# ViV99/slam-experiments

Hardware: NVIDIA B200
Metric: hamming_pairs_per_sec (higher is better)
Workload: dtype u8

## Files before the change

### slam_experiments_b200/csrc/hm_tc.cu

```cuda
#include <math.h>
#include <stdlib.h>

#include <mutex>
#include <type_traits>

#include <cuda_fp16.h>

#include "hm_common.cuh"
#include "hm_tcgen05.cuh"

#ifndef HM_F4_TILE_N
#define HM_F4_TILE_N 128
#endif

namespace hm {

namespace {

constexpr int kRowBlock = 128;
constexpr int kMBlocks = 2;
constexpr int kBlockM = kRowBlock * kMBlocks;
constexpr int kSlabBytes = kRowBlock * 128;
constexpr int kPadRows = HM_PREPARED_TILE_ROWS;
constexpr int kTmemCols = 512;
constexpr uint32_t kSpinLimit = 1u << 26;

static_assert(kPadRows % kBlockM == 0, "prepared padding must cover whole query blocks");

struct CoreI8 {
    using Acc = int;
    static constexpr int kSlabs = 2;
    static constexpr int kRowBytes = HM_PREPARED_ROW_BYTES;
    static constexpr int kTileN = 128;
    static constexpr int kStages = 4;
    static constexpr int kUnits = 4;
    static constexpr int kColSplit = 1;
    static constexpr bool kRegisterHandover = false;
    static constexpr bool kScales = false;
    static constexpr int kPrologueTiles = 45;
    static __device__ __forceinline__ Acc lowest() { return INT_MIN; }
    static __device__ __forceinline__ Acc from_bits(uint32_t x) { return (int)x; }
    static __device__ __forceinline__ Acc max3(Acc a, Acc b, Acc c) { return __vimax3_s32(a, b, c); }
    static __device__ __forceinline__ Acc max2(Acc a, Acc b) { return max(a, b); }
    static __device__ __forceinline__ bool valid(Acc v) { return v >= -256; }
    static __device__ __forceinline__ unsigned distance(Acc v) { return (unsigned)((256 - v) >> 1); }
    static __device__ __forceinline__ unsigned encode(Acc v) { return (unsigned)(v + 257); }
    static __device__ __forceinline__ Acc floor_from(unsigned e) { return (int)e - 259; }
    static __device__ __forceinline__ uint32_t pack2(uint32_t lo, uint32_t hi) { return ((uint32_t)max((int)lo, -32768) & 0xFFFFu) | ((uint32_t)max((int)hi, -32768) << 16); }
    static __device__ __forceinline__ Acc unpack(uint32_t p, int hi) { return hi ? (int)p >> 16 : (int)(short)(p & 0xFFFFu); }
    static constexpr uint32_t kLowestBits = 0x80000000u;
};

struct CoreF4 {
    using Acc = float;
    static constexpr int kSlabs = 1;
    static constexpr int kRowBytes = HM_PREPARED_F4_ROW_BYTES;
    static constexpr int kTileN = HM_F4_TILE_N;
#ifndef HM_F4_STAGES
#define HM_F4_STAGES 6
#endif
    static constexpr int kStages = HM_F4_TILE_N == 96 ? 10 : HM_F4_TILE_N == 64 ? 14 : HM_F4_STAGES;
#ifndef HM_F4_UNITS
#define HM_F4_UNITS (HM_F4_TILE_N == 96 ? 5 : HM_F4_TILE_N == 64 ? 7 : 3)
#endif
    static constexpr int kUnits = HM_F4_UNITS;
    static constexpr int kColSplit = 2;
    static constexpr bool kRegisterHandover = true;
    static constexpr bool kScales = true;
    static constexpr int kPrologueTiles = 90;
    static __device__ __forceinline__ Acc lowest() { return -INFINITY; }
    static __device__ __forceinline__ Acc from_bits(uint32_t x) { return __uint_as_float(x); }
    static __device__ __forceinline__ Acc max3(Acc a, Acc b, Acc c) { return fmaxf(fmaxf(a, b), c); }
    static __device__ __forceinline__ Acc max2(Acc a, Acc b) { return fmaxf(a, b); }
    static __device__ __forceinline__ bool valid(Acc v) { return v >= -256.0f; }
    static __device__ __forceinline__ unsigned distance(Acc v) { return (unsigned)((256 - (int)v) >> 1); }
    static __device__ __forceinline__ unsigned encode(Acc v) { return (unsigned)((int)v + 257); }
    static __device__ __forceinline__ Acc floor_from(unsigned e) { return (float)((int)e - 259); }
    static __device__ __forceinline__ uint32_t pack2(uint32_t lo, uint32_t hi)
    {
        const __half2 h = __floats2half2_rn(__uint_as_float(lo), __uint_as_float(hi));
        return *reinterpret_cast<const uint32_t*>(&h);
    }
    static __device__ __forceinline__ Acc unpack(uint32_t p, int hi)
    {
        const __half2 h = *reinterpret_cast<const __half2*>(&p);
        return hi ? __high2float(h) : __low2float(h);
    }
    static constexpr uint32_t kLowestBits = 0xFF800000u;
};

template <class C> __host__ __device__ constexpr int row_block_bytes() { return kRowBlock * C::kRowBytes; }
template <class C> __host__ __device__ constexpr int a_bytes() { return kMBlocks * row_block_bytes<C>(); }
template <class C> __host__ __device__ constexpr int b_stage_bytes() { return C::kTileN * C::kRowBytes; }
template <class C> __host__ __device__ constexpr int epilogue_warps() { return 4 * kMBlocks * C::kColSplit; }
template <class C> __host__ __device__ constexpr int control_warps() { return C::kRegisterHandover ? 4 : 2; }
template <class C> __host__ __device__ constexpr int threads() { return 32 * (control_warps<C>() + epilogue_warps<C>()); }
constexpr int kHandoverBytes = kBlockM * 16;
constexpr int kBarrierBytes = 512;
template <class C> __host__ __device__ constexpr int smem_bytes() { return 1024 + a_bytes<C>() + C::kStages * b_stage_bytes<C>() + kBarrierBytes + kHandoverBytes; }
static_assert((2 * CoreF4::kStages + 1 + 2 * CoreF4::kUnits) * 8 + 16 <= kBarrierBytes, "barrier block");
static_assert((2 * CoreI8::kStages + 1 + 2 * CoreI8::kUnits) * 8 + 16 <= kBarrierBytes, "barrier block");
__host__ __device__ constexpr int ct_gcd(int a, int b) { return b == 0 ? a : ct_gcd(b, a % b); }
template <class C> __host__ __device__ constexpr int issuer_period() { return C::kStages / ct_gcd(C::kStages, C::kUnits) * C::kUnits; }
constexpr int kScaleCols = 32;
constexpr int kScaleCol = kTmemCols - kScaleCols;
static_assert(CoreF4::kUnits * CoreF4::kTileN <= kScaleCol, "accumulator units must end before the scale factors");

struct PrepareParams {
    const uint8_t* bits;
    long long n, stride, batch_stride;
    long long padded_rows;
    uint8_t* out;
};

__global__ void __launch_bounds__(256) hm_prepare_kernel(const PrepareParams P)
{
    const long long chunks_per_problem = P.padded_rows * 16;
    const long long o = (long long)blockIdx.x * blockDim.x + threadIdx.x;
    if (o >= chunks_per_problem) return;
    const int b = blockIdx.y;
    const long long rb = o >> 11;
    const int rem = (int)(o & 2047);
    const int slab = rem >> 10;
    const int rem2 = rem & 1023;
    const int rr = (rem2 >> 3) & 7;
    const int r = ((rem2 >> 6) << 3) | rr;
    const int c = (rem2 & 7) ^ rr;
// ... 130 lines not shown
#if HM_TC_TRACE
    unsigned slow;
#endif
};

__device__ __forceinline__ void bounded_wait(uint64_t* bar, uint32_t parity, int* error_flag)
{
    uint32_t spins = 0;
    while (!ptx::mbar_try_wait(bar, parity)) {
        if (++spins > kSpinLimit) {
            if (error_flag) atomicExch(error_flag, 1);
            __trap();
        }
    }
}

__device__ __forceinline__ void bounded_wait_addr(uint32_t bar_addr, uint32_t parity, int* error_flag)
{
    uint32_t spins = 0;
    while (!ptx::mbar_try_wait_addr(bar_addr, parity)) {
        if (++spins > kSpinLimit) {
            if (error_flag) atomicExch(error_flag, 1);
            __trap();
        }
    }
}

#define HM_R8(a, o) "+r"(a[o]), "+r"(a[o + 1]), "+r"(a[o + 2]), "+r"(a[o + 3]), "+r"(a[o + 4]), "+r"(a[o + 5]), "+r"(a[o + 6]), "+r"(a[o + 7])
#define HM_R32(a) HM_R8(a, 0), HM_R8(a, 8), HM_R8(a, 16), HM_R8(a, 24)
__device__ __forceinline__ void tmem_ld_fence4(uint32_t (&a)[32], uint32_t (&b)[32], uint32_t (&c)[32], uint32_t (&d)[32])
{
    asm volatile("tcgen05.wait::ld.sync.aligned;\n" : HM_R32(a), HM_R32(b), HM_R32(c), HM_R32(d) : : "memory");
}
__device__ __forceinline__ void tmem_ld_fence48(uint32_t (&a)[32], uint32_t (&b)[16])
{
    asm volatile("tcgen05.wait::ld.sync.aligned;\n" : HM_R32(a), HM_R8(b, 0), HM_R8(b, 8) : : "memory");
}
__device__ __forceinline__ void tmem_ld_fence64(uint32_t (&a)[64])
{
    asm volatile("tcgen05.wait::ld.sync.aligned;\n" : HM_R8(a, 0), HM_R8(a, 8), HM_R8(a, 16), HM_R8(a, 24), HM_R8(a, 32), HM_R8(a, 40), HM_R8(a, 48), HM_R8(a, 56) : : "memory");
}

template <class C, int kMode, int kGroups = 4>
__device__ __forceinline__ void scan_chunk(const uint32_t* r, unsigned colbase, Top2<typename C::Acc>& s)
{
    using Acc = typename C::Acc;
    static_assert(kGroups == 2 || kGroups == 4 || kGroups == 8, "8-column groups per compare");
    Acc gm[kGroups];
#pragma unroll
    for (int g = 0; g < kGroups; ++g) {
        const int o = g * 8;
        gm[g] = C::max3(C::max3(C::from_bits(r[o]), C::from_bits(r[o + 1]), C::from_bits(r[o + 2])),
                        C::max3(C::from_bits(r[o + 3]), C::from_bits(r[o + 4]), C::from_bits(r[o + 5])),
                        C::max2(C::from_bits(r[o + 6]), C::from_bits(r[o + 7])));
    }
    Acc m;
    if constexpr (kGroups == 8) m = C::max3(C::max3(gm[0], gm[1], gm[2]), C::max3(gm[3], gm[4], gm[5]), C::max2(gm[6], gm[7]));
    else if constexpr (kGroups == 4) m = C::max3(gm[0], gm[1], C::max2(gm[2], gm[3]));
    else m = C::max2(gm[0], gm[1]);
    constexpr bool kFloor = kMode == 1, kTop1 = kMode == 2;
    if (m > (kFloor ? s.f : kTop1 ? s.v1 : s.v2)) {
#if HM_TC_TRACE
        s.slow += 1;
#endif
#pragma unroll
        for (int g = 0; g < kGroups; ++g) {
            const Acc x = gm[g];
            if (x > (kFloor ? s.f : kTop1 ? s.v1 : s.v2)) {
                const int o = g * 8;
                const uint32_t p0 = C::pack2(r[o], r[o + 1]), p1 = C::pack2(r[o + 2], r[o + 3]);
                const uint32_t p2 = C::pack2(r[o + 4], r[o + 5]), p3 = C::pack2(r[o + 6], r[o + 7]);
                const unsigned idx = colbase + o;
                if (kTop1 || x > s.v1) {
                    if (!kTop1) {
                        s.v2 = s.v1; s.i2 = s.i1;
                        s.sb[0] = s.sa[0]; s.sb[1] = s.sa[1]; s.sb[2] = s.sa[2]; s.sb[3] = s.sa[3];
                    }
                    s.v1 = x; s.i1 = idx;
                    s.sa[0] = p0; s.sa[1] = p1; s.sa[2] = p2; s.sa[3] = p3;
                } else {
                    s.v2 = x; s.i2 = idx;
                    s.sb[0] = p0; s.sb[1] = p1; s.sb[2] = p2; s.sb[3] = p3;
                }
                if (kFloor) s.f = C::max2(s.v2, s.f);
            }
        }
    }
}

template <class C, int kN>
__device__ __forceinline__ void mask_tail(uint32_t* r, unsigned colbase, unsigned limit)
{
    if (colbase + kN > limit) {
#pragma unroll
        for (int j = 0; j < kN; ++j)
            if (colbase + j >= limit) r[j] = C::kLowestBits;
    }
}

#ifndef HM_ARRIVE_ELECT
#define HM_ARRIVE_ELECT 1
#endif
#ifndef HM_SCAN_FLAT64
#define HM_SCAN_FLAT64 1
#endif
#ifndef HM_FLOOR_DENSE_TILES
#define HM_FLOOR_DENSE_TILES 32
#endif
#ifndef HM_FLOOR_LATE_MASK
#define HM_FLOOR_LATE_MASK 15
#endif

#ifndef HM_F4_A_TMEM
#define HM_F4_A_TMEM 0
#endif
constexpr int kATmemCol = 384;
constexpr int kATmemColsPerBlock = 32;

template <class C>
__device__ __forceinline__ void issue_half(int h, uint32_t a_block, uint32_t b_stage, uint32_t tmem_d, uint32_t idesc,
                                           uint32_t tmem_sf)
{
    constexpr int kHalf = C::kSlabs * 2;
#pragma unroll
    for (int jj = 0; jj < kHalf; ++jj) {
        const int j = h * kHalf + jj;
        const int slab = j >> 2, k = j & 3;
        const uint64_t db = ptx::kmajor_sw128_desc_from_lo(b_stage + ((slab * kSlabBytes + k * 32) >> 4));
        if constexpr (C::kScales && HM_F4_A_TMEM) {
            ptx::mma_mxf4_ts(tmem_d, a_block + 8 * j, db, idesc, tmem_sf, tmem_sf + kScaleCols / 2, j != 0);
        } else {
            const uint64_t da = ptx::kmajor_sw128_desc_from_lo(a_block + ((slab * kSlabBytes + k * 32) >> 4));
            if constexpr (C::kScales) ptx::mma_mxf4_ss(tmem_d, da, db, idesc, tmem_sf, tmem_sf + kScaleCols / 2, j != 0);
            else                      ptx::mma_i8_ss(tmem_d, da, db, idesc, j != 0);
        }
    }
}

// ... 21 lines not shown
    uint64_t* tmem_empty_bar = tmem_full_bar + kUnits;
    uint32_t* tmem_base_slot = reinterpret_cast<uint32_t*>(tmem_empty_bar + kUnits);
    uint32_t* smem_base_slot = tmem_base_slot + 2;
    ulonglong2* handover = reinterpret_cast<ulonglong2*>(smem + kABytes + kStages * kBStageBytes + kBarrierBytes);

    const int warp = __shfl_sync(0xffffffffu, threadIdx.x >> 5, 0);
    const int lane = threadIdx.x & 31;
    if (threadIdx.x == 0) cta_mark(P, 0);
    if (threadIdx.x == 0 && (blockIdx.x | blockIdx.y | blockIdx.z) == 0 && P.clock_probe) {
        unsigned long long t;
        asm volatile("mov.u64 %0, %%globaltimer;" : "=l"(t));
        P.clock_probe[0] = (long long)t;
        P.clock_probe[1] = clock64();
    }
    const int qb = blockIdx.x;
    const int split = blockIdx.y;
    const int b = blockIdx.z;

    const uint32_t cs = ptx::cluster_nctarank();
    const uint32_t crank = ptx::cluster_ctarank();
    const uint16_t cmask = (uint16_t)((1u << cs) - 1);
    const bool has_a = qb < P.q_blocks_valid;
    auto rows_present = [&]() -> long long { return P.nq_dyn ? min((long long)__ldg(P.nq_dyn + b), P.nq) : P.nq; };
    if (P.nq_dyn && (long long)(qb - (int)crank) * kBlockM >= rows_present()) return;

    const int tile_begin = split * P.tiles_per_split;
    const int tile_end = min(tile_begin + P.tiles_per_split, P.ntiles);
    const int my_tiles = tile_end - tile_begin;

    constexpr int kProducerWarp = kIssuerLast ? epilogue_warps<C>() : 0;
    constexpr int kIssuerWarp = kIssuerLast ? epilogue_warps<C>() + 1 : 1;
    constexpr int kFirstEpiWarp = kIssuerLast ? 0 : 2;
    static_assert(kIssuerLast || !C::kRegisterHandover, "the control warps must form the last warpgroup");
    static_assert(!C::kRegisterHandover || (epilogue_warps<C>() == 16 && threads<C>() == 640),
                  "the register budget (4 x 32 + 16 x 112 = 20 x 96) assumes 20 warps launched at 96 registers");
    if (warp == kProducerWarp && lane == 0) {
        *smem_base_slot = ptx::smem_u32(smem);
        for (int i = 0; i < kStages; ++i) {
            ptx::mbar_init(&full_bar[i], 1);
            ptx::mbar_init(&empty_bar[i], cs);
        }
        ptx::mbar_init(a_full_bar, 1);
        for (int i = 0; i < kUnits; ++i) {
            ptx::mbar_init(&tmem_full_bar[i], 1);
            ptx::mbar_init(&tmem_empty_bar[i], 4 * C::kColSplit);
        }
        ptx::fence_barrier_init();
        ptx::fence_proxy_async();
    } else if (warp == kIssuerWarp) {
        ptx::tmem_alloc(tmem_base_slot, kTmemCols);
        ptx::tmem_relinquish();
    }
    ptx::tc_fence_before();
    if (cs > 1) ptx::cluster_sync();
    else __syncthreads();
    ptx::tc_fence_after();
    const uint32_t tmem_base = *tmem_base_slot;

    if constexpr (C::kScales) {
        if (warp >= kFirstEpiWarp && warp < kFirstEpiWarp + 4) {
            uint32_t ones[32];
#pragma unroll
            for (int i = 0; i < 32; ++i) ones[i] = 0x7F7F7F7Fu;
            const uint32_t taddr = tmem_base + ((uint32_t)((warp & 3) * 32) << 16) + kScaleCol;
            static_assert(kScaleCols == 32, "one x32 store per lane quarter");
            ptx::tmem_st_32x32(taddr, ones);
            ptx::tmem_st_wait();
        }
// ... 27 lines not shown
                            const uint4 v = row[c ^ (r & 7)];
                            words[4 * c] = v.x; words[4 * c + 1] = v.y; words[4 * c + 2] = v.z; words[4 * c + 3] = v.w;
                        }
                    }
                }
                ptx::tmem_st_32x32(tmem_base + ((uint32_t)(wq * 32) << 16) + kATmemCol + wblk * kATmemColsPerBlock, words);
                ptx::tmem_st_wait();
            }
        } else if (P.qbits) {
            const uint8_t* qsrc = P.qbits + (long long)b * P.q_bits_batch_stride;
            const int* qidx = P.q_index ? P.q_index + (long long)b * P.q_index_batch_stride : nullptr;
            const long long nq_eff = rows_present();
            for (int o = threadIdx.x; o < kBlockM * 8; o += blockDim.x) {
                const int blk = o >> 10, rem = o & 1023;
                const int rr = (rem >> 3) & 7;
                const int r = ((rem >> 6) << 3) | rr;
                const int c = (rem & 7) ^ rr;
                const long long qrow = (long long)qb * kBlockM + blk * kRowBlock + r;
                uint4 v = make_uint4(0, 0, 0, 0);
                if (qrow < nq_eff) {
                    const long long srow = qidx ? (long long)__ldg(qidx + qrow) : qrow;
                    v = expand_bits_e2m1(*reinterpret_cast<const unsigned*>(qsrc + srow * P.q_bits_stride + c * 4));
                }
                reinterpret_cast<uint4*>(smem_a)[o] = v;
            }
            ptx::fence_proxy_async();
        }
        ptx::tc_fence_before();
        __syncthreads();
        ptx::tc_fence_after();
    }

    if (threadIdx.x == 0) cta_mark(P, 1);
    ulonglong2 my_keys = make_ulonglong2(kNoMatch, kNoMatch);
    long long my_row = -1;
    int my_row_in_cta = 0;

    auto run_producer = [&]() {
        if (lane == 0) {
            if (has_a && !P.qbits && !(C::kScales && HM_F4_A_TMEM)) {
                const uint8_t* qsrc = P.qprep + ((long long)b * P.q_padded + (long long)qb * kBlockM) * C::kRowBytes;
                ptx::mbar_arrive_expect_tx(a_full_bar, kABytes);
                ptx::bulk_g2s(smem_a, qsrc, kABytes, a_full_bar);
            }
            const uint8_t* tsrc = P.tprep + (long long)b * P.t_padded * C::kRowBytes;
            const uint32_t piece = kBStageBytes / cs;
            for (int i = 0; i < (HM_TC_EXPERIMENT >= 5 ? 0 : my_tiles); ++i) {
                const int stage = i % kStages;
                const uint32_t use = i / kStages;
#if HM_TC_EXPERIMENT < 4
                bounded_wait(&empty_bar[stage], (use & 1) ^ 1, P.error_flag);
#endif
                trace_mark(P, i, 0);
                ptx::mbar_arrive_expect_tx(&full_bar[stage], kBStageBytes);
                uint8_t* dst = smem_b + stage * kBStageBytes + crank * piece;
                const uint8_t* src = tsrc + (long long)(tile_begin + i) * kBStageBytes + crank * piece;
                if (cs > 1) ptx::bulk_g2s_multicast(dst, src, piece, &full_bar[stage], cmask);
                else        ptx::bulk_g2s(dst, src, piece, &full_bar[stage]);
            }
        }
    };
    auto run_issuer = [&]() {
        const bool leader = ptx::elect_one();
        const uint32_t idesc = C::kScales ? ptx::make_mxf4_idesc(kRowBlock, kTileN) : ptx::make_i8_idesc(kRowBlock, kTileN);
        constexpr bool kATmem = C::kScales && HM_F4_A_TMEM;
        const uint32_t a_addr = kATmem ? tmem_base + kATmemCol : ptx::smem_u32(smem_a) >> 4;
        constexpr uint32_t kABlockStep = kATmem ? (uint32_t)kATmemColsPerBlock : (uint32_t)(kRowBlockBytes >> 4);
        const uint32_t b_addr = ptx::smem_u32(smem_b) >> 4;
        const uint32_t tmem_sf = tmem_base + kScaleCol;
// ... 41 lines not shown
                    if (leader) issue_half<C>(0, a_addr + kABlockStep, b_stage, tmem_base + unit_b * kTileN, idesc, tmem_sf);
                    ready0 = false;
                    if (base + j + 1 < my_tiles) {
                        const int n = j + 1;
#if HM_TC_EXPERIMENT >= 4
                        ready0 = true;
#else
                        ready0 = __all_sync(0xffffffffu,
                                            ptx::mbar_test_wait(&full_bar[n % kStages], sphase ^ ((n / kStages) & 1))
#if HM_TC_EXPERIMENT < 3
                                            && ptx::mbar_test_wait(&tmem_empty_bar[(2 * n) % kUnits], (((2 * n) / kUnits) & 1) ^ 1)
#endif
                                            );
#endif
                    }
                    if (leader) {
                        issue_half<C>(1, a_addr + kABlockStep, b_stage, tmem_base + unit_b * kTileN, idesc, tmem_sf);
#if HM_TC_EXPERIMENT == 6 || HM_COMMIT_MODE == 1
                        ptx::tc_commit(&tmem_full_bar[unit_a]);
#endif
                        ptx::tc_commit(&tmem_full_bar[unit_b]);
                        if (cs > 1) ptx::tc_commit_multicast(&empty_bar[stage], cmask);
                        else        ptx::tc_commit(&empty_bar[stage]);
                    }
                }
            }
            sphase ^= (kPeriod / kStages) & 1;
        }
        __syncwarp();
    };
    auto run_epilogue = [&]() {
        constexpr int kCols = kTileN / C::kColSplit;
        const int quarter = warp & 3;
        const int mblk = ((warp - kFirstEpiWarp) >> 2) & 1;
        const int half = (warp - kFirstEpiWarp) >> 3;
        const int row_in_cta = mblk * kRowBlock + quarter * 32 + lane;
        const long long row = (long long)qb * kBlockM + row_in_cta;
        Top2<Acc> s;
        s.v1 = s.v2 = C::lowest();
        s.i1 = s.i2 = 0;
#pragma unroll
        for (int e = 0; e < 4; ++e) s.sa[e] = s.sb[e] = 0;
        s.f = C::floor_from(0);
#if HM_TC_TRACE
        s.slow = 0;
#endif
        unsigned floor_code = 0;
        const long long first_row = (long long)tile_begin * kTileN;
        const unsigned limit = (unsigned)min((long long)my_tiles * kTileN, P.nt - first_row);
        const uint32_t bars_addr = ptx::lds_volatile_u32(ptx::smem_u32(smem_base_slot)) + kABytes + kStages * kBStageBytes;
        const uint32_t unit_full_addr = bars_addr + (2 * kStages + 1) * 8;
        const uint32_t unit_empty_addr = unit_full_addr + kUnits * 8;
        int unit = mblk;
        uint32_t unit_use = 0;
        unsigned floor_pending = 0;
        auto refresh_floor = [&](int i) {
            if constexpr (kFloor) {
                if (i < HM_FLOOR_DENSE_TILES || (i & HM_FLOOR_LATE_MASK) == 0) {
                    floor_code = max(floor_code, floor_pending);
                    s.f = C::max2(s.f, C::floor_from(floor_code));
                    if (row < P.nq) {
                        unsigned* floor_ptr = P.row_floor + ((long long)b * P.nq + row);
                        const unsigned e = C::valid(s.v2) ? C::encode(s.v2) : 0u;
                        if (e > floor_code) { atomicMax(floor_ptr, e); floor_code = e; }
                        floor_pending = __ldcg(floor_ptr);
                    }
                }
            }
        };
        auto process_tile = [&](int i) {
            bounded_wait_addr(unit_full_addr + unit * 8, unit_use & 1, P.error_flag);
#if HM_TC_TRACE == 2
            if (warp == kFirstEpiWarp && lane == 0 && (i == 8 || i == 32 || i == 64 || i == 192)) cta_mark(P, i == 8 ? 5 : i == 32 ? 6 : i == 64 ? 7 : 8);
#endif
            if (warp == kFirstEpiWarp && lane == 0) trace_mark(P, i, 3);
            if (warp == kFirstEpiWarp + 7 && lane == 0) trace_mark(P, i, 5);
            ptx::tc_fence_after();
            const uint32_t taddr = tmem_base + ((uint32_t)(quarter * 32) << 16) + unit * kTileN + half * kCols;
            const unsigned colbase = (unsigned)i * kTileN + half * kCols;
            if constexpr (C::kColSplit == 1) {
                uint32_t r0[32], r1[32], r2[32], r3[32];
                ptx::tmem_ld_32x32(taddr, r0);
                ptx::tmem_ld_32x32(taddr + 32, r1);
                ptx::tmem_ld_32x32(taddr + 64, r2);
                ptx::tmem_ld_32x32(taddr + 96, r3);
                refresh_floor(i);
                tmem_ld_fence4(r0, r1, r2, r3);
                ptx::tc_fence_before();
                __syncwarp();
                if (HM_ARRIVE_ELECT ? ptx::elect_one() : lane == 0) ptx::mbar_arrive_addr(unit_empty_addr + unit * 8);
                if (colbase + kCols > limit) {
                    mask_tail<C, 32>(r0, colbase, limit);
                    mask_tail<C, 32>(r1, colbase + 32, limit);
                    mask_tail<C, 32>(r2, colbase + 64, limit);
                    mask_tail<C, 32>(r3, colbase + 96, limit);
                }
                scan_chunk<C, kMode>(r0, colbase, s);
                scan_chunk<C, kMode>(r1, colbase + 32, s);
                scan_chunk<C, kMode>(r2, colbase + 64, s);
                scan_chunk<C, kMode>(r3, colbase + 96, s);
            } else {
                if constexpr (kCols == 64) {
                    uint32_t r[64];
#if HM_TC_EXPERIMENT < 2
                    ptx::tmem_ld_32x64(taddr, r);
                    refresh_floor(i);
                    tmem_ld_fence64(r);
#endif
                    ptx::tc_fence_before();
                    __syncwarp();
                    if (HM_ARRIVE_ELECT ? ptx::elect_one() : lane == 0) ptx::mbar_arrive_addr(unit_empty_addr + unit * 8);
#if HM_TC_EXPERIMENT != 0
                    unit += 2;
                    if (unit >= kUnits) { unit -= kUnits; ++unit_use; }
                    return;
#endif
                    mask_tail<C, 64>(r, colbase, limit);
#if HM_SCAN_FLAT64
                    scan_chunk<C, kMode, 8>(r, colbase, s);
#else
                    scan_chunk<C, kMode>(r, colbase, s);
                    scan_chunk<C, kMode>(r + 32, colbase + 32, s);
#endif
                } else if constexpr (kCols == 32) {
                    uint32_t r[32];
                    ptx::tmem_ld_32x32(taddr, r);
                    refresh_floor(i);
                    asm volatile("tcgen05.wait::ld.sync.aligned;\n" : HM_R32(r) : : "memory");
                    ptx::tc_fence_before();
                    __syncwarp();
                    if (HM_ARRIVE_ELECT ? ptx::elect_one() : lane == 0) ptx::mbar_arrive_addr(unit_empty_addr + unit * 8);
                    mask_tail<C, 32>(r, colbase, limit);
                    scan_chunk<C, kMode>(r, colbase, s);
                } else {
                    static_assert(kCols == 64 || kCols == 48, "column split");
                    uint32_t r0[32], r1[16];
                    ptx::tmem_ld_32x32(taddr, r0);
                    ptx::tmem_ld_32x16(taddr + 32, r1);
                    refresh_floor(i);
                    tmem_ld_fence48(r0, r1);
                    ptx::tc_fence_before();
                    __syncwarp();
                    if (HM_ARRIVE_ELECT ? ptx::elect_one() : lane == 0) ptx::mbar_arrive_addr(unit_empty_addr + unit * 8);
                    mask_tail<C, 32>(r0, colbase, limit);
                    mask_tail<C, 16>(r1, colbase + 32, limit);
                    scan_chunk<C, kMode>(r0, colbase, s);
                    scan_chunk<C, kMode, 2>(r1, colbase + 32, s);
                }
            }
            unit += 2;
            if (unit >= kUnits) { unit -= kUnits; ++unit_use; }
            if (warp == kFirstEpiWarp && lane == 0) trace_mark(P, i, 4);
        };
#pragma unroll 1
        for (int i = 0; i < my_tiles; ++i) process_tile(i);
        if (warp == kFirstEpiWarp && lane == 0) cta_mark(P, 2);
#if HM_TC_TRACE
        if (P.trace) {
            const long long cta = ((long long)blockIdx.z * gridDim.y + blockIdx.y) * gridDim.x + blockIdx.x;
            long long* rec = P.trace + kTraceTiles * kTraceSlots + cta * kCtaSlots;
            const unsigned any = __reduce_max_sync(0xffffffffu, s.slow);
            const unsigned sum = __reduce_add_sync(0xffffffffu, s.slow);
            if (lane == 0) { atomicAdd((unsigned long long*)&rec[9], (unsigned long long)any); atomicAdd((unsigned long long*)&rec[10], (unsigned long long)sum); }
        }
#endif
        const unsigned long long gbase = P.train_base + (unsigned long long)first_row;
        auto fold_group = [&](Acc v, unsigned i0, const uint32_t (&p)[4]) {
            if (!C::valid(v)) return;
#pragma unroll
            for (int e = 0; e < 8; ++e) {
                const Acc x = C::unpack(p[e >> 1], e & 1);
                if (C::valid(x)) top2_insert(my_keys.x, my_keys.y, ((unsigned long long)C::distance(x) << 32) | (gbase + i0 + e));
            }
        };
        fold_group(s.v1, s.i1, s.sa);
        if (kMode != 2) fold_group(s.v2, s.i2, s.sb);
        else my_keys.y = kNoMatch;
        if (half == 1) handover[row_in_cta] = my_keys;
        else my_row = row;
        my_row_in_cta = row_in_cta;
    };

    auto run_tail = [&](auto worker_tag) {
        constexpr bool kWorker = decltype(worker_tag)::value;
        ptx::tc_fence_before();
        if (cs > 1) ptx::cluster_sync();
        else __syncthreads();
        if (kWorker && threadIdx.x == 0) cta_mark(P, 3);
        if (warp == kIssuerWarp) {
            ptx::tc_fence_after();
            ptx::tmem_dealloc(tmem_base, kTmemCols);
        }
        if (kWorker && my_row >= 0 && my_row < rows_present()) {
            if constexpr (C::kColSplit == 2) {
                const ulonglong2 o = handover[my_row_in_cta];
                top2_insert(my_keys.x, my_keys.y, o.x);
                top2_insert(my_keys.x, my_keys.y, o.y);
            }
            unsigned long long* out = P.out + (long long)split * P.out_split_stride + ((long long)b * P.nq + my_row) * 2;
            *reinterpret_cast<ulonglong2*>(out) = my_keys;
            if (!P.counters) select_candidate(P.sel, b, my_keys);
        }
        if (P.counters) {
            int* flag = reinterpret_cast<int*>(tmem_base_slot + 1);
            if (last_cta_arrives(&P.counters[(long long)b * gridDim.x + qb], (unsigned)P.splits, flag)) {
                const long long row = (long long)qb * kBlockM + threadIdx.x;
                const bool has_row = kWorker && threadIdx.x < kBlockM && row < rows_present();
                ulonglong2 k = make_ulonglong2(kNoMatch, kNoMatch);
                if (has_row) fold_partials(P.out, P.splits, P.out_split_stride, (long long)b * P.nq + row, k.x, k.y);
                if (P.xch.world > 1 && (long long)qb * kBlockM < P.nq) k = exchange_and_merge(P.xch, row, has_row, k, qb);
                if (has_row) {
                    *reinterpret_cast<ulonglong2*>(P.final_out + ((long long)b * P.nq + row) * 2) = k;
                    select_candidate(P.sel, b, k);
                }
            }
        }
        if (kWorker && threadIdx.x == 0) cta_mark(P, 4);
        if (kWorker && threadIdx.x == 0 && (blockIdx.x | blockIdx.y | blockIdx.z) == 0 && P.clock_probe) {
            unsigned long long t;
            asm volatile("mov.u64 %0, %%globaltimer;" : "=l"(t));
            P.clock_probe[2] = (long long)t;
            P.clock_probe[3] = clock64();
        }
    };

    if constexpr (C::kRegisterHandover) {
        if (warp >= kProducerWarp) {
            asm volatile("setmaxnreg.dec.sync.aligned.u32 32;\n");
            if (warp == kProducerWarp) run_producer();
            else if (warp == kIssuerWarp) run_issuer();
            run_tail(std::false_type{});
            return;
        }
        asm volatile("setmaxnreg.inc.sync.aligned.u32 112;\n");
        run_epilogue();
        run_tail(std::true_type{});
    } else {
        if (warp == kProducerWarp) run_producer();
        else if (warp == kIssuerWarp) run_issuer();
        else run_epilogue();
        run_tail(std::true_type{});
    }
}

__global__ void __launch_bounds__(threads<CoreI8>(), 1) hm_i8_knn2_kernel(const TcParams P) { tc_knn2_body<CoreI8, 0>(P); }
__global__ void __launch_bounds__(threads<CoreF4>(), 1) hm_f4_knn2_kernel(const TcParams P) { tc_knn2_body<CoreF4, 0>(P); }
__global__ void __launch_bounds__(threads<CoreI8>(), 1) hm_i8_knn2_floor_kernel(const TcParams P) { tc_knn2_body<CoreI8, 1>(P); }
__global__ void __launch_bounds__(threads<CoreF4>(), 1) hm_f4_knn2_floor_kernel(const TcParams P) { tc_knn2_body<CoreF4, 1>(P); }
__global__ void __launch_bounds__(threads<CoreI8>(), 1) hm_i8_knn1_kernel(const TcParams P) { tc_knn2_body<CoreI8, 2>(P); }
__global__ void __launch_bounds__(threads<CoreF4>(), 1) hm_f4_knn1_kernel(const TcParams P) { tc_knn2_body<CoreF4, 2>(P); }

using KernelFn = void (*)(const TcParams);
template <class C> KernelFn kernel_of(int mode = 0);
template <> KernelFn kernel_of<CoreI8>(int mode) { return mode == 1 ? hm_i8_knn2_floor_kernel : mode == 2 ? hm_i8_knn1_kernel : hm_i8_knn2_kernel; }
template <> KernelFn kernel_of<CoreF4>(int mode) { return mode == 1 ? hm_f4_knn2_floor_kernel : mode == 2 ? hm_f4_knn1_kernel : hm_f4_knn2_kernel; }

struct TcPlan {
    int ntiles, splits, tiles_per_split;
    int cluster;
    long long qblocks;
};

int floor_max_tiles()
{
    static int v = -1;
    if (v < 0) {
        const char* e = getenv("HM_FLOOR_MAX_TILES");
// ... 278 lines not shown
    if (le != cudaSuccess) {
        set_error("cudaLaunchKernelEx(tensor-core k-NN kernel, cluster %d) failed: %s", pl.cluster, cudaGetErrorString(le));
        return HM_ERR_CUDA;
    }
    HM_CUDA_CHECK(cudaGetLastError());
    if (trace_path) {
        static long long host[kTraceTiles * kTraceSlots];
        HM_CUDA_CHECK(cudaStreamSynchronize(stream));
        HM_CUDA_CHECK(cudaMemcpy(host, P.trace, sizeof(host), cudaMemcpyDeviceToHost));
        {
            const size_t nctas = (size_t)pl.qblocks * pl.splits * batch;
            long long* rec = (long long*)malloc(nctas * kCtaSlots * sizeof(long long));
            if (rec && cudaMemcpy(rec, P.trace + kTraceTiles * kTraceSlots, nctas * kCtaSlots * sizeof(long long), cudaMemcpyDeviceToHost) == cudaSuccess) {
                char path[1024];
                snprintf(path, sizeof(path), "%s.ctas", trace_path);
                if (FILE* f = fopen(path, "w")) {
                    fprintf(f, "# cta entry_ns prologue_done loop_done final_barrier exit tile8 tile32 tile64 tile192 smid slow_warp_chunks_lb slow_lane_chunks (globaltimer ns since the first entry); grid=(%lld,%d,%d)\n", pl.qblocks, pl.splits, batch);
                    long long t0 = -1;
                    for (size_t c = 0; c < nctas; ++c) if (rec[c * kCtaSlots] && (t0 < 0 || rec[c * kCtaSlots] < t0)) t0 = rec[c * kCtaSlots];
                    for (size_t c = 0; c < nctas; ++c) {
                        fprintf(f, "%zu", c);
                        for (int k = 0; k < 9; ++k) fprintf(f, " %lld", rec[c * kCtaSlots + k] ? rec[c * kCtaSlots + k] - t0 : -1);
                        fprintf(f, " %lld %lld %lld", rec[c * kCtaSlots + 11], rec[c * kCtaSlots + 9], rec[c * kCtaSlots + 10]);
                        for (int k = 0; k < 9; ++k) fprintf(f, " %lld", rec[c * kCtaSlots + 12 + k] ? rec[c * kCtaSlots + 12 + k] - rec[c * kCtaSlots + 12] : -1);
                        fprintf(f, "\n");
                    }
                    fclose(f);
                }
            }
            free(rec);
        }
        cudaFree(P.trace);
        if (FILE* f = fopen(trace_path, "w")) {
            fprintf(f, "# tile producer_issue issuer_ready (unused) epi2_full epi2_scanned epi9_full issuer_unit1_free issuer_loop_top (cycles since first stamp); tiles/CTA=%d splits=%d cluster=%d core=%s\n",
                    pl.tiles_per_split, pl.splits, pl.cluster, C::kScales ? "mxf4" : "i8");
            long long t0 = host[0];
            for (int i = 0; i < kTraceTiles; ++i) {
                fprintf(f, "%d", i + P.trace_first);
                for (int k = 0; k < 8; ++k) fprintf(f, " %lld", host[i * kTraceSlots + k] ? host[i * kTraceSlots + k] - t0 : -1);
                fprintf(f, "\n");
            }
            fclose(f);
        }
    }
    if (keep_partials) {
        if (out_partials) *out_partials = partials;
        if (out_groups) *out_groups = pl.splits;
    }
    return HM_OK;
}

template <class C>
int launch_prepare_of(const uint8_t* bits, long long n, long long stride, long long batch_stride, int batch,
                      void* prepared, cudaStream_t stream)
{
    if (n <= 0 || batch <= 0) return HM_OK;
    PrepareParams P{};
    P.bits = bits; P.n = n; P.stride = stride; P.batch_stride = batch_stride;
    P.padded_rows = padded_rows<C>(n);
    P.out = static_cast<uint8_t*>(prepared);
    const long long chunks = P.padded_rows * (C::kRowBytes / 16);
    dim3 grid((unsigned)ceil_div(chunks, 256), (unsigned)batch);
    if (C::kScales) hm_prepare_f4_kernel<<<grid, 256, 0, stream>>>(P);
    else            hm_prepare_kernel<<<grid, 256, 0, stream>>>(P);
    HM_CUDA_CHECK(cudaGetLastError());
    return HM_OK;
}
// ... 135 lines not shown
```

Before: 13840.

## Have each F4 epilogue warp scan both query blocks with double-buffered TMEM loads

For the MXF4 core, epilogue warps drop from 16 to 8. Each warp now covers both 128-row query blocks, alternating between two 64-column register buffers so the next TMEM load overlaps the scan of the current one. The register budget per epilogue warp rises from 112 to 232 to hold two buffers and two top-2 states. The tile-size and unit macros are removed. The change trades warp-level parallelism for software pipelining inside each warp, which reduces launch occupancy and could leave TMEM drain slower if one warp cannot keep up with the MMA.

```diff
diff --git a/slam_experiments_b200/csrc/hm_tc.cu b/slam_experiments_b200/csrc/hm_tc.cu
--- a/slam_experiments_b200/csrc/hm_tc.cu
+++ b/slam_experiments_b200/csrc/hm_tc.cu
@@ -8,10 +8,6 @@
 
 #include "hm_common.cuh"
 #include "hm_tcgen05.cuh"
-
-#ifndef HM_F4_TILE_N
-#define HM_F4_TILE_N 128
-#endif
 
 namespace hm {
 
@@ -35,6 +31,7 @@
     static constexpr int kStages = 4;
     static constexpr int kUnits = 4;
     static constexpr int kColSplit = 1;
+    static constexpr bool kBothBlocks = false;
     static constexpr bool kRegisterHandover = false;
     static constexpr bool kScales = false;
     static constexpr int kPrologueTiles = 45;
@@ -55,16 +52,14 @@
     using Acc = float;
     static constexpr int kSlabs = 1;
     static constexpr int kRowBytes = HM_PREPARED_F4_ROW_BYTES;
-    static constexpr int kTileN = HM_F4_TILE_N;
+    static constexpr int kTileN = 128;
 #ifndef HM_F4_STAGES
 #define HM_F4_STAGES 6
 #endif
-    static constexpr int kStages = HM_F4_TILE_N == 96 ? 10 : HM_F4_TILE_N == 64 ? 14 : HM_F4_STAGES;
-#ifndef HM_F4_UNITS
-#define HM_F4_UNITS (HM_F4_TILE_N == 96 ? 5 : HM_F4_TILE_N == 64 ? 7 : 3)
-#endif
-    static constexpr int kUnits = HM_F4_UNITS;
+    static constexpr int kStages = HM_F4_STAGES;
+    static constexpr int kUnits = 3;
     static constexpr int kColSplit = 2;
+    static constexpr bool kBothBlocks = true;
     static constexpr bool kRegisterHandover = true;
     static constexpr bool kScales = true;
     static constexpr int kPrologueTiles = 90;
@@ -92,7 +87,7 @@
 template <class C> __host__ __device__ constexpr int row_block_bytes() { return kRowBlock * C::kRowBytes; }
 template <class C> __host__ __device__ constexpr int a_bytes() { return kMBlocks * row_block_bytes<C>(); }
 template <class C> __host__ __device__ constexpr int b_stage_bytes() { return C::kTileN * C::kRowBytes; }
-template <class C> __host__ __device__ constexpr int epilogue_warps() { return 4 * kMBlocks * C::kColSplit; }
+template <class C> __host__ __device__ constexpr int epilogue_warps() { return 4 * (C::kBothBlocks ? 1 : kMBlocks) * C::kColSplit; }
 template <class C> __host__ __device__ constexpr int control_warps() { return C::kRegisterHandover ? 4 : 2; }
 template <class C> __host__ __device__ constexpr int threads() { return 32 * (control_warps<C>() + epilogue_warps<C>()); }
 constexpr int kHandoverBytes = kBlockM * 16;
@@ -289,13 +284,12 @@
 {
     asm volatile("tcgen05.wait::ld.sync.aligned;\n" : HM_R32(a), HM_R32(b), HM_R32(c), HM_R32(d) : : "memory");
 }
-__device__ __forceinline__ void tmem_ld_fence48(uint32_t (&a)[32], uint32_t (&b)[16])
-{
-    asm volatile("tcgen05.wait::ld.sync.aligned;\n" : HM_R32(a), HM_R8(b, 0), HM_R8(b, 8) : : "memory");
-}
-__device__ __forceinline__ void tmem_ld_fence64(uint32_t (&a)[64])
-{
-    asm volatile("tcgen05.wait::ld.sync.aligned;\n" : HM_R8(a, 0), HM_R8(a, 8), HM_R8(a, 16), HM_R8(a, 24), HM_R8(a, 32), HM_R8(a, 40), HM_R8(a, 48), HM_R8(a, 56) : : "memory");
+__device__ __forceinline__ void tmem_ld_fence64_after(uint32_t (&a)[64], Top2<float>& s)
+{
+    asm volatile("tcgen05.wait::ld.sync.aligned;\n"
+                 : HM_R8(a, 0), HM_R8(a, 8), HM_R8(a, 16), HM_R8(a, 24), HM_R8(a, 32), HM_R8(a, 40), HM_R8(a, 48), HM_R8(a, 56),
+                   "+f"(s.v1), "+f"(s.v2), "+f"(s.f)
+                 : : "memory");
 }
 
 template <class C, int kMode, int kGroups = 4>
@@ -358,9 +352,6 @@
 #ifndef HM_ARRIVE_ELECT
 #define HM_ARRIVE_ELECT 1
 #endif
-#ifndef HM_SCAN_FLAT64
-#define HM_SCAN_FLAT64 1
-#endif
 #ifndef HM_FLOOR_DENSE_TILES
 #define HM_FLOOR_DENSE_TILES 32
 #endif
@@ -448,8 +439,8 @@
     constexpr int kIssuerWarp = kIssuerLast ? epilogue_warps<C>() + 1 : 1;
     constexpr int kFirstEpiWarp = kIssuerLast ? 0 : 2;
     static_assert(kIssuerLast || !C::kRegisterHandover, "the control warps must form the last warpgroup");
-    static_assert(!C::kRegisterHandover || (epilogue_warps<C>() == 16 && threads<C>() == 640),
-                  "the register budget (4 x 32 + 16 x 112 = 20 x 96) assumes 20 warps launched at 96 registers");
+    static_assert(!C::kRegisterHandover || (epilogue_warps<C>() == 8 && threads<C>() == 384 && 4 * 32 + 8 * 232 <= 12 * 168),
+                  "the register budget (4 x 32 + 8 x 232 <= 12 x 168) assumes 12 warps launched at 168 registers");
     if (warp == kProducerWarp && lane == 0) {
         *smem_base_slot = ptx::smem_u32(smem);
         for (int i = 0; i < kStages; ++i) {
@@ -543,9 +534,16 @@
     }
 
     if (threadIdx.x == 0) cta_mark(P, 1);
-    ulonglong2 my_keys = make_ulonglong2(kNoMatch, kNoMatch);
-    long long my_row = -1;
-    int my_row_in_cta = 0;
+    constexpr int kBlocks = C::kBothBlocks ? kMBlocks : 1;
+    ulonglong2 my_keys[kBlocks];
+    long long my_row[kBlocks];
+    int my_row_in_cta[kBlocks];
+#pragma unroll
+    for (int k = 0; k < kBlocks; ++k) {
+        my_keys[k] = make_ulonglong2(kNoMatch, kNoMatch);
+        my_row[k] = -1;
+        my_row_in_cta[k] = 0;
+    }
 
     auto run_producer = [&]() {
         if (lane == 0) {
@@ -653,153 +651,168 @@
     auto run_epilogue = [&]() {
         constexpr int kCols = kTileN / C::kColSplit;
         const int quarter = warp & 3;
-        const int mblk = ((warp - kFirstEpiWarp) >> 2) & 1;
-        const int half = (warp - kFirstEpiWarp) >> 3;
-        const int row_in_cta = mblk * kRowBlock + quarter * 32 + lane;
-        const long long row = (long long)qb * kBlockM + row_in_cta;
-        Top2<Acc> s;
-        s.v1 = s.v2 = C::lowest();
-        s.i1 = s.i2 = 0;
-#pragma unroll
-        for (int e = 0; e < 4; ++e) s.sa[e] = s.sb[e] = 0;
-        s.f = C::floor_from(0);
+        const int mblk0 = C::kBothBlocks ? 0 : ((warp - kFirstEpiWarp) >> 2) & 1;
+        const int half = (warp - kFirstEpiWarp) / (4 * (C::kBothBlocks ? 1 : kMBlocks));
+        long long row[kBlocks];
+        Top2<Acc> s[kBlocks];
+        unsigned floor_code[kBlocks], floor_pending[kBlocks];
+#pragma unroll
+        for (int k = 0; k < kBlocks; ++k) {
+            my_row_in_cta[k] = (mblk0 + k) * kRowBlock + quarter * 32 + lane;
+            row[k] = (long long)qb * kBlockM + my_row_in_cta[k];
+            s[k].v1 = s[k].v2 = C::lowest();
+            s[k].i1 = s[k].i2 = 0;
+#pragma unroll
+            for (int e = 0; e < 4; ++e) s[k].sa[e] = s[k].sb[e] = 0;
+            s[k].f = C::floor_from(0);
 #if HM_TC_TRACE
-        s.slow = 0;
-#endif
-        unsigned floor_code = 0;
+            s[k].slow = 0;
+#endif
+            floor_code[k] = 0;
+            floor_pending[k] = 0;
+        }
         const long long first_row = (long long)tile_begin * kTileN;
         const unsigned limit = (unsigned)min((long long)my_tiles * kTileN, P.nt - first_row);
         const uint32_t bars_addr = ptx::lds_volatile_u32(ptx::smem_u32(smem_base_slot)) + kABytes + kStages * kBStageBytes;
         const uint32_t unit_full_addr = bars_addr + (2 * kStages + 1) * 8;
         const uint32_t unit_empty_addr = unit_full_addr + kUnits * 8;
-        int unit = mblk;
-        uint32_t unit_use = 0;
-        unsigned floor_pending = 0;
-        auto refresh_floor = [&](int i) {
+        auto refresh_floor = [&](int k, int i) {
             if constexpr (kFloor) {
                 if (i < HM_FLOOR_DENSE_TILES || (i & HM_FLOOR_LATE_MASK) == 0) {
-                    floor_code = max(floor_code, floor_pending);
-                    s.f = C::max2(s.f, C::floor_from(floor_code));
-                    if (row < P.nq) {
-                        unsigned* floor_ptr = P.row_floor + ((long long)b * P.nq + row);
-                        const unsigned e = C::valid(s.v2) ? C::encode(s.v2) : 0u;
-                        if (e > floor_code) { atomicMax(floor_ptr, e); floor_code = e; }
-                        floor_pending = __ldcg(floor_ptr);
+                    floor_code[k] = max(floor_code[k], floor_pending[k]);
+                    s[k].f = C::max2(s[k].f, C::floor_from(floor_code[k]));
+                    if (row[k] < P.nq) {
+                        unsigned* floor_ptr = P.row_floor + ((long long)b * P.nq + row[k]);
+                        const unsigned e = C::valid(s[k].v2) ? C::encode(s[k].v2) : 0u;
+                        if (e > floor_code[k]) { atomicMax(floor_ptr, e); floor_code[k] = e; }
+                        floor_pending[k] = __ldcg(floor_ptr);
                     }
                 }
             }
         };
-        auto process_tile = [&](int i) {
+        int unit = mblk0;
+        uint32_t unit_use = 0;
+        auto next_unit = [&](int step) {
+            unit += step;
+            if (unit >= kUnits) { unit -= kUnits; ++unit_use; }
+        };
+        auto unit_taddr = [&]() { return tmem_base + ((uint32_t)(quarter * 32) << 16) + unit * kTileN + half * kCols; };
+        auto wait_unit_full = [&]() {
             bounded_wait_addr(unit_full_addr + unit * 8, unit_use & 1, P.error_flag);
+            ptx::tc_fence_after();
+        };
+        auto release_unit = [&]() {
+            ptx::tc_fence_before();
+            __syncwarp();
+            if (HM_ARRIVE_ELECT ? ptx::elect_one() : lane == 0) ptx::mbar_arrive_addr(unit_empty_addr + unit * 8);
+        };
+        if constexpr (C::kBothBlocks) {
+            static_assert(kCols == 64 && kBlocks == 2, "two 64-column buffers, one per query block");
+            const bool stamp = warp == kFirstEpiWarp && lane == 0;
+            uint32_t r0[64], r1[64];
+            wait_unit_full();
+            if (stamp) trace_mark(P, 0, 3);
+            ptx::tmem_ld_32x64(unit_taddr(), r0);
+            tmem_ld_fence64_after(r0, s[0]);
+            release_unit();
+            if (stamp) trace_mark(P, 0, 4);
+            next_unit(1);
+#pragma unroll 1
+            for (int i = 0; i < my_tiles; ++i) {
 #if HM_TC_TRACE == 2
-            if (warp == kFirstEpiWarp && lane == 0 && (i == 8 || i == 32 || i == 64 || i == 192)) cta_mark(P, i == 8 ? 5 : i == 32 ? 6 : i == 64 ? 7 : 8);
-#endif
-            if (warp == kFirstEpiWarp && lane == 0) trace_mark(P, i, 3);
-            if (warp == kFirstEpiWarp + 7 && lane == 0) trace_mark(P, i, 5);
-            ptx::tc_fence_after();
-            const uint32_t taddr = tmem_base + ((uint32_t)(quarter * 32) << 16) + unit * kTileN + half * kCols;
-            const unsigned colbase = (unsigned)i * kTileN + half * kCols;
-            if constexpr (C::kColSplit == 1) {
+                if (stamp && (i == 8 || i == 32 || i == 64 || i == 192)) cta_mark(P, i == 8 ? 5 : i == 32 ? 6 : i == 64 ? 7 : 8);
+#endif
+                const unsigned colbase = (unsigned)i * kTileN + half * kCols;
+                wait_unit_full();
+                if (stamp) trace_mark(P, i, 5);
+                ptx::tmem_ld_32x64(unit_taddr(), r1);
+                refresh_floor(0, i);
+                mask_tail<C, 64>(r0, colbase, limit);
+                scan_chunk<C, kMode, 8>(r0, colbase, s[0]);
+                tmem_ld_fence64_after(r1, s[0]);
+                release_unit();
+                if (stamp) trace_mark(P, i, 2);
+                next_unit(1);
+                const bool more = i + 1 < my_tiles;
+                if (more) {
+                    wait_unit_full();
+                    if (stamp) trace_mark(P, i + 1, 3);
+                    ptx::tmem_ld_32x64(unit_taddr(), r0);
+                }
+                refresh_floor(1, i);
+                mask_tail<C, 64>(r1, colbase, limit);
+                scan_chunk<C, kMode, 8>(r1, colbase, s[1]);
+                if (more) {
+                    tmem_ld_fence64_after(r0, s[1]);
+                    release_unit();
+                    if (stamp) trace_mark(P, i + 1, 4);
+                    next_unit(1);
+                }
+            }
+        } else {
+            static_assert(C::kColSplit == 1, "one warp per (query block, lane quarter) scans whole tiles");
+#pragma unroll 1
+            for (int i = 0; i < my_tiles; ++i) {
+#if HM_TC_TRACE == 2
+                if (warp == kFirstEpiWarp && lane == 0 && (i == 8 || i == 32 || i == 64 || i == 192)) cta_mark(P, i == 8 ? 5 : i == 32 ? 6 : i == 64 ? 7 : 8);
+#endif
+                wait_unit_full();
+                if (warp == kFirstEpiWarp && lane == 0) trace_mark(P, i, 3);
+                if (warp == kFirstEpiWarp + 7 && lane == 0) trace_mark(P, i, 5);
+                const uint32_t taddr = unit_taddr();
+                const unsigned colbase = (unsigned)i * kTileN;
                 uint32_t r0[32], r1[32], r2[32], r3[32];
                 ptx::tmem_ld_32x32(taddr, r0);
                 ptx::tmem_ld_32x32(taddr + 32, r1);
                 ptx::tmem_ld_32x32(taddr + 64, r2);
                 ptx::tmem_ld_32x32(taddr + 96, r3);
-                refresh_floor(i);
+                refresh_floor(0, i);
                 tmem_ld_fence4(r0, r1, r2, r3);
-                ptx::tc_fence_before();
-                __syncwarp();
-                if (HM_ARRIVE_ELECT ? ptx::elect_one() : lane == 0) ptx::mbar_arrive_addr(unit_empty_addr + unit * 8);
+                release_unit();
                 if (colbase + kCols > limit) {
                     mask_tail<C, 32>(r0, colbase, limit);
                     mask_tail<C, 32>(r1, colbase + 32, limit);
                     mask_tail<C, 32>(r2, colbase + 64, limit);
                     mask_tail<C, 32>(r3, colbase + 96, limit);
                 }
-                scan_chunk<C, kMode>(r0, colbase, s);
-                scan_chunk<C, kMode>(r1, colbase + 32, s);
-                scan_chunk<C, kMode>(r2, colbase + 64, s);
-                scan_chunk<C, kMode>(r3, colbase + 96, s);
-            } else {
-                if constexpr (kCols == 64) {
-                    uint32_t r[64];
-#if HM_TC_EXPERIMENT < 2
-                    ptx::tmem_ld_32x64(taddr, r);
-                    refresh_floor(i);
-                    tmem_ld_fence64(r);
-#endif
-                    ptx::tc_fence_before();
-                    __syncwarp();
-                    if (HM_ARRIVE_ELECT ? ptx::elect_one() : lane == 0) ptx::mbar_arrive_addr(unit_empty_addr + unit * 8);
-#if HM_TC_EXPERIMENT != 0
-                    unit += 2;
-                    if (unit >= kUnits) { unit -= kUnits; ++unit_use; }
-                    return;
-#endif
-                    mask_tail<C, 64>(r, colbase, limit);
-#if HM_SCAN_FLAT64
-                    scan_chunk<C, kMode, 8>(r, colbase, s);
-#else
-                    scan_chunk<C, kMode>(r, colbase, s);
-                    scan_chunk<C, kMode>(r + 32, colbase + 32, s);
-#endif
-                } else if constexpr (kCols == 32) {
-                    uint32_t r[32];
-                    ptx::tmem_ld_32x32(taddr, r);
-                    refresh_floor(i);
-                    asm volatile("tcgen05.wait::ld.sync.aligned;\n" : HM_R32(r) : : "memory");
-                    ptx::tc_fence_before();
-                    __syncwarp();
-                    if (HM_ARRIVE_ELECT ? ptx::elect_one() : lane == 0) ptx::mbar_arrive_addr(unit_empty_addr + unit * 8);
-                    mask_tail<C, 32>(r, colbase, limit);
-                    scan_chunk<C, kMode>(r, colbase, s);
-                } else {
-                    static_assert(kCols == 64 || kCols == 48, "column split");
-                    uint32_t r0[32], r1[16];
-                    ptx::tmem_ld_32x32(taddr, r0);
-                    ptx::tmem_ld_32x16(taddr + 32, r1);
-                    refresh_floor(i);
-                    tmem_ld_fence48(r0, r1);
-                    ptx::tc_fence_before();
-                    __syncwarp();
-                    if (HM_ARRIVE_ELECT ? ptx::elect_one() : lane == 0) ptx::mbar_arrive_addr(unit_empty_addr + unit * 8);
-                    mask_tail<C, 32>(r0, colbase, limit);
-                    mask_tail<C, 16>(r1, colbase + 32, limit);
-                    scan_chunk<C, kMode>(r0, colbase, s);
-                    scan_chunk<C, kMode, 2>(r1, colbase + 32, s);
-                }
+                scan_chunk<C, kMode>(r0, colbase, s[0]);
+                scan_chunk<C, kMode>(r1, colbase + 32, s[0]);
+                scan_chunk<C, kMode>(r2, colbase + 64, s[0]);
+                scan_chunk<C, kMode>(r3, colbase + 96, s[0]);
+                next_unit(2);
+                if (warp == kFirstEpiWarp && lane == 0) trace_mark(P, i, 4);
             }
-            unit += 2;
-            if (unit >= kUnits) { unit -= kUnits; ++unit_use; }
-            if (warp == kFirstEpiWarp && lane == 0) trace_mark(P, i, 4);
-        };
-#pragma unroll 1
-        for (int i = 0; i < my_tiles; ++i) process_tile(i);
+        }
         if (warp == kFirstEpiWarp && lane == 0) cta_mark(P, 2);
 #if HM_TC_TRACE
         if (P.trace) {
+            unsigned slow = 0;
+#pragma unroll
+            for (int k = 0; k < kBlocks; ++k) slow += s[k].slow;
             const long long cta = ((long long)blockIdx.z * gridDim.y + blockIdx.y) * gridDim.x + blockIdx.x;
             long long* rec = P.trace + kTraceTiles * kTraceSlots + cta * kCtaSlots;
-            const unsigned any = __reduce_max_sync(0xffffffffu, s.slow);
-            const unsigned sum = __reduce_add_sync(0xffffffffu, s.slow);
+            const unsigned any = __reduce_max_sync(0xffffffffu, slow);
+            const unsigned sum = __reduce_add_sync(0xffffffffu, slow);
             if (lane == 0) { atomicAdd((unsigned long long*)&rec[9], (unsigned long long)any); atomicAdd((unsigned long long*)&rec[10], (unsigned long long)sum); }
         }
 #endif
         const unsigned long long gbase = P.train_base + (unsigned long long)first_row;
-        auto fold_group = [&](Acc v, unsigned i0, const uint32_t (&p)[4]) {
-            if (!C::valid(v)) return;
-#pragma unroll
-            for (int e = 0; e < 8; ++e) {
-                const Acc x = C::unpack(p[e >> 1], e & 1);
-                if (C::valid(x)) top2_insert(my_keys.x, my_keys.y, ((unsigned long long)C::distance(x) << 32) | (gbase + i0 + e));
-            }
-        };
-        fold_group(s.v1, s.i1, s.sa);
-        if (kMode != 2) fold_group(s.v2, s.i2, s.sb);
-        else my_keys.y = kNoMatch;
-        if (half == 1) handover[row_in_cta] = my_keys;
-        else my_row = row;
-        my_row_in_cta = row_in_cta;
+#pragma unroll
+        for (int k = 0; k < kBlocks; ++k) {
+            auto fold_group = [&](Acc v, unsigned i0, const uint32_t (&p)[4]) {
+                if (!C::valid(v)) return;
+#pragma unroll
+                for (int e = 0; e < 8; ++e) {
+                    const Acc x = C::unpack(p[e >> 1], e & 1);
+                    if (C::valid(x)) top2_insert(my_keys[k].x, my_keys[k].y, ((unsigned long long)C::distance(x) << 32) | (gbase + i0 + e));
+                }
+            };
+            fold_group(s[k].v1, s[k].i1, s[k].sa);
+            if (kMode != 2) fold_group(s[k].v2, s[k].i2, s[k].sb);
+            else my_keys[k].y = kNoMatch;
+            if (half == 1) handover[my_row_in_cta[k]] = my_keys[k];
+            else my_row[k] = row[k];
+        }
     };
 
     auto run_tail = [&](auto worker_tag) {
@@ -812,15 +825,18 @@
             ptx::tc_fence_after();
             ptx::tmem_dealloc(tmem_base, kTmemCols);
         }
-        if (kWorker && my_row >= 0 && my_row < rows_present()) {
-            if constexpr (C::kColSplit == 2) {
-                const ulonglong2 o = handover[my_row_in_cta];
-                top2_insert(my_keys.x, my_keys.y, o.x);
-                top2_insert(my_keys.x, my_keys.y, o.y);
+#pragma unroll
+        for (int k = 0; k < kBlocks; ++k) {
+            if (kWorker && my_row[k] >= 0 && my_row[k] < rows_present()) {
+                if constexpr (C::kColSplit == 2) {
+                    const ulonglong2 o = handover[my_row_in_cta[k]];
+                    top2_insert(my_keys[k].x, my_keys[k].y, o.x);
+                    top2_insert(my_keys[k].x, my_keys[k].y, o.y);
+                }
+                unsigned long long* out = P.out + (long long)split * P.out_split_stride + ((long long)b * P.nq + my_row[k]) * 2;
+                *reinterpret_cast<ulonglong2*>(out) = my_keys[k];
+                if (!P.counters) select_candidate(P.sel, b, my_keys[k]);
             }
-            unsigned long long* out = P.out + (long long)split * P.out_split_stride + ((long long)b * P.nq + my_row) * 2;
-            *reinterpret_cast<ulonglong2*>(out) = my_keys;
-            if (!P.counters) select_candidate(P.sel, b, my_keys);
         }
         if (P.counters) {
             int* flag = reinterpret_cast<int*>(tmem_base_slot + 1);
@@ -853,7 +869,7 @@
             run_tail(std::false_type{});
             return;
         }
-        asm volatile("setmaxnreg.inc.sync.aligned.u32 112;\n");
+        asm volatile("setmaxnreg.inc.sync.aligned.u32 232;\n");
         run_epilogue();
         run_tail(std::true_type{});
     } else {
@@ -1198,7 +1214,7 @@
         }
         cudaFree(P.trace);
         if (FILE* f = fopen(trace_path, "w")) {
-            fprintf(f, "# tile producer_issue issuer_ready (unused) epi2_full epi2_scanned epi9_full issuer_unit1_free issuer_loop_top (cycles since first stamp); tiles/CTA=%d splits=%d cluster=%d core=%s\n",
+            fprintf(f, "# tile producer_issue issuer_ready epi_unit1_released epi_unit0_full epi_unit0_released(mxf4)/scanned(i8) epi_unit1_full issuer_unit1_free issuer_loop_top (cycles since first stamp); tiles/CTA=%d splits=%d cluster=%d core=%s\n",
                     pl.tiles_per_split, pl.splits, pl.cluster, C::kScales ? "mxf4" : "i8");
             long long t0 = host[0];
             for (int i = 0; i < kTraceTiles; ++i) {
```

New measurement: 8907 (median of 6 runs). 0.644x the previous value.
